# MisterPup/PDE-MultiGrid

Hardware: AMD Instinct MI355X
Metric: MLUPS on 3D Poisson 512^3 V-cycle (higher is better)
Workload: dtype f64

## Files before the change

include/mgx.h:

```cpp
#ifndef MGX_H
#define MGX_H

#include <stddef.h>
#include <stdint.h>

#ifdef __cplusplus
extern "C" {
#endif

typedef enum {
    MGX_OK = 0,
    MGX_ERR_INVALID = 1,
    MGX_ERR_SIZE = 2,
    MGX_ERR_HIP = 3,
    MGX_ERR_NOMEM = 4,
    MGX_ERR_RCCL = 5,
    MGX_ERR_NOGPU = 6
} mgx_status;

typedef enum { MGX_RESIDUAL_REF_COMPAT = 0, MGX_RESIDUAL_CORRECT = 1 } mgx_residual_mode;

typedef struct mgx_ctx mgx_ctx;
typedef struct mgx_event mgx_event;

const char* mgx_status_string(int status);
const char* mgx_last_error(void);
void mgx_set_last_error(const char* msg);
const char* mgx_version(void);

int mgx_device_count(int* count);
int mgx_ctx_create(int device, mgx_ctx** out);
int mgx_ctx_destroy(mgx_ctx* ctx);
int mgx_ctx_sync(mgx_ctx* ctx);
int mgx_ctx_check(mgx_ctx* ctx);
int mgx_ctx_clear_abort(mgx_ctx* ctx, int reenable);
int mgx_ctx_generation(const mgx_ctx* ctx, unsigned long long* generation);
int mgx_ctx_prepare(mgx_ctx* ctx);
int mgx_ctx_device(const mgx_ctx* ctx, int* device);
int mgx_ctx_set_param(mgx_ctx* ctx, const char* name, int value);
const char* mgx_ctx_last_relax_kernel(const mgx_ctx* ctx);
const char* mgx_ctx_last_rr_kernel(const mgx_ctx* ctx);
const char* mgx_ctx_last_corr_kernel(const mgx_ctx* ctx);
const char* mgx_ctx_last_block3_kernel(const mgx_ctx* ctx);
int mgx3dxs_relax_block3_f64(mgx_ctx* ctx, const double* vin, double* vout, const double* f, const int n[3], const double h[3],
                             int first_colour, int store_both);
int mgx3dxs_relax_block3_corr_f64(mgx_ctx* ctx, double* v, const double* f, const int n[3], const double h[3], const double* coarse_v,
                                  const int cn[3]);
int mgx_test_set_lds_poison(int on);
int mgx_test_lds_probe(mgx_ctx* ctx, double* fraction);
int mgx_ctx_stream(const mgx_ctx* ctx, void** hip_stream);

int mgx_malloc(mgx_ctx* ctx, size_t bytes, void** dptr);
int mgx_free(mgx_ctx* ctx, void* dptr);
int mgx_memcpy_h2d(mgx_ctx* ctx, void* dst, const void* host_src, size_t bytes);
int mgx_memcpy_d2h(mgx_ctx* ctx, void* host_dst, const void* src, size_t bytes);
int mgx_memcpy_d2d(mgx_ctx* ctx, void* dst, const void* src, size_t bytes);
int mgx_memset_zero(mgx_ctx* ctx, void* dst, size_t bytes);

int mgx_graph_begin(mgx_ctx* ctx);
int mgx_graph_end(mgx_ctx* ctx, void** graph_exec);
int mgx_graph_launch(mgx_ctx* ctx, void* graph_exec);
int mgx_graph_destroy(mgx_ctx* ctx, void* graph_exec);
int mgx_event_create(mgx_ctx* ctx, mgx_event** out);
int mgx_event_destroy(mgx_ctx* ctx, mgx_event* ev);
int mgx_event_record(mgx_ctx* ctx, mgx_event* ev);
int mgx_event_elapsed_ms(mgx_ctx* ctx, mgx_event* start, mgx_event* stop, float* ms);

#define MGX_DECLARE_OPS(SFX, real)                                                                      \
    int mgx3d_relax_##SFX(mgx_ctx* ctx, real* v, const real* f, const int n[3], const real h[3],        \
                          int ncycles);                                                                 \
     \
     \
     \
    int mgx3d_relax_from_zero_##SFX(mgx_ctx* ctx, real* v, const real* f, const int n[3], const real h[3], \
                                    int ncycles, int rim_is_zero);                                      \
    int mgx3d_residual_##SFX(mgx_ctx* ctx, const real* v, const real* f, real* r, const int n[3],       \
                             const real h[3], int mode);                                                \
    int mgx3d_restrict_##SFX(mgx_ctx* ctx, const real* fine, const int fn[3], real* coarse,             \
                             const int cn[3]);                                                          \
    int mgx3d_interpolate_##SFX(mgx_ctx* ctx, real* fine, const int fn[3], const real* coarse,          \
// ... 497 lines not shown
```

pde_multigrid_amd/csrc/mgx_block3d.hip:

```cpp
#include <type_traits>

#include "mgx_host3d.hpp"

namespace mgx {

template <class real, int COL, bool STORE_BOTH, int TW, bool CORR = false>
__global__ void __launch_bounds__(64 * TW, 4)
    relax3d_xs_block3_kernel(const real* vin, real* vout, const real* __restrict__ f, int sx, int sy, int sz, real hx2, real hy2,
                             real hz2, int zrun, int gx, int gy, int xcd_mode, const real* coarse = nullptr, int cx = 0,
                             int cy = 0) {
    constexpr int ROWS = 2 * TW, OUTR = ROWS - 6;
    static_assert(OUTR % 2 == 0, "the colour parity of a wave's rows must not depend on the tile");
    static_assert(!CORR || (COL == 0 && !STORE_BOTH), "the correcting variant is R', B, R with red stored");
    __shared__ real sY[2][TW][2][64];
    __shared__ real sX[2][TW][2][64];
    __shared__ real sZ[2][TW][2][64];
    const Geo<XSplit, real> g(sx, sy);
    const int lane = threadIdx.x;
    const int w = __builtin_amdgcn_readfirstlane(threadIdx.y);
    int bx, by, bz;
    tile_of_block(xcd_mode, gx, gy, bx, by, bz);
    const int z0 = 1 + bz * zrun, z1 = min(z0 + zrun, sz - 1);
    if (z0 >= z1) return;
    const int PL = (int)g.PL;

    const int Hn = (sx + 1) >> 1;
    const int pn = bx * 60 + lane - 2, p = min(max(pn, 0), Hn - 1);
    const unsigned off0 = (unsigned)p * (unsigned)sizeof(real), off1 = (unsigned)(g.H + (p <= Hn - 2 ? p : 0)) * (unsigned)sizeof(real);
    const bool xin0 = pn >= 1 && 2 * pn <= sx - 2, xin1 = pn >= 0 && 2 * pn + 1 <= sx - 2;
    auto off = [&](int h) { return h ? off1 : off0; };
    auto xin = [&](int h) { return h ? xin1 : xin0; };
    const bool xface0 = pn <= 0 || pn >= Hn - 1;
    const bool wxface = bx * 60 - 2 <= 0 || bx * 60 + 61 >= Hn - 1;
    const bool outlane = lane >= 2 && lane <= 61;
    int roff[2];
    bool yin[2], outrow[2];
#pragma unroll
    for (int o = 0; o < 2; o++) {
        const int y = by * OUTR - 3 + 2 * w + o;
        roff[o] = min(max(y, 0), sy - 1) * g.P;
        yin[o] = y >= 1 && y <= sy - 2;
        outrow[o] = 2 * w + o >= 3 && 2 * w + o < ROWS - 3;
    }
    const int wU = w > 0 ? w - 1 : 0, wD = w < TW - 1 ? w + 1 : TW - 1;
    auto zc = [&](int z) { return min(max(z, 0), sz - 1); };
    auto plane = [&](const real* a, int z) { return plane_rsrc<real>(a + (ptrdiff_t)zc(z) * (ptrdiff_t)g.PL, PL, 1); };
    const Geo<XSplit, real> gc(CORR ? cx : 3, CORR ? cy : 3);
    const int cz = (sz + 1) >> 1;
    int croff[2];
#pragma unroll
    for (int i = 0; i < 2; i++) croff[i] = CORR ? min(max(by * (OUTR / 2) - 2 + w + i, 0), cy - 1) * gc.P : 0;
    const unsigned coff = (unsigned)XSplit::pos(p, gc.H) * (unsigned)sizeof(real);
    auto cplane = [&](int k) {
        return plane_rsrc<real>(coarse + (ptrdiff_t)min(max(k, 0), cz - 1) * (ptrdiff_t)gc.PL, (int)gc.PL, 1);
    };
    auto interp = [&](int ox, int oz, int o, const real (&k0)[2], const real (&k1)[2]) __attribute__((always_inline)) {
        return interpolate3d_point<real>(ox, 1 - o, oz, [&](int dx, int dy, int dz) __attribute__((always_inline)) {
            const real c = o + dy ? (dz ? k1[1] : k0[1]) : (dz ? k1[0] : k0[0]);
            return dx ? wave_from_next_lane<real>(c) : c;
        });
    };

    real a_m[2], a_c[2], a_p[2], a_n[2], fx_c[2], fx_1[2], fx_2[2], fx_n[2], xv_n[2], fy_c[2], fy_n[2];
    real b_c[2], b_m[2], b_mm[2], d_c[2], d_m[2], d_mm[2], x3[2];
    real c_0[2], c_1[2], c_n[2], e_n[2];
#pragma unroll
    for (int o = 0; o < 2; o++)
        a_m[o] = a_c[o] = a_p[o] = a_n[o] = fx_c[o] = fx_1[o] = fx_2[o] = fx_n[o] = xv_n[o] = fy_c[o] = fy_n[o] = b_c[o] =
            b_m[o] = b_mm[o] = d_c[o] = d_m[o] = d_mm[o] = x3[o] = c_0[o] = c_1[o] = c_n[o] = e_n[o] = 0;

    const int t0 = z0 - 2, tlast = z1 + 1;
    {
        const auto qm = plane(vin, t0 - 1), q0 = plane(vin, t0), qp = plane(vin, t0 + 1);
        const bool zf = t0 <= 0 || t0 >= sz - 1;
        const auto qf = plane(f, t0);
#pragma unroll
        for (int o = 0; o < 2; o++) {
            const int hx = (COL + 1 + o + t0) & 1;
            a_m[o] = buf_load<real>(qm, off(hx), roff[o]);
            a_c[o] = buf_load<real>(q0, off(hx ^ 1), roff[o]);
            a_p[o] = buf_load<real>(qp, off(hx), roff[o]);
            fx_c[o] = buf_load<real>(zf || !yin[o] ? q0 : qf, off(hx), roff[o]);
            if (wxface) xv_n[o] = buf_load<real>(q0, off(0), roff[o]);
        }
        __builtin_amdgcn_s_waitcnt(0x0F70);
#pragma unroll
        for (int o = 0; o < 2; o++)
            if (wxface && ((COL + 1 + o + t0) & 1) == 0 && xface0) fx_c[o] = xv_n[o];
        if constexpr (CORR) {
#pragma unroll
            for (int d = -1; d <= 1; d++) {
                const int z = t0 + d;
                const auto k0q = cplane(z >> 1), k1q = cplane((z >> 1) + 1);
                real k0[2], k1[2];
#pragma unroll
                for (int i = 0; i < 2; i++) {
                    k0[i] = buf_load<real>(k0q, coff, croff[i]);
                    k1[i] = buf_load<real>(k1q, coff, croff[i]);
                }
                const bool zin = z >= 1 && z <= sz - 2;
#pragma unroll
                for (int o = 0; o < 2; o++) {
                    const int hb = (COL + o + z) & 1;
                    const real e = interp(hb, z & 1, o, k0, k1);
                    real& a = d < 0 ? a_m[o] : d == 0 ? a_c[o] : a_p[o];
// ... 13 lines not shown
        const int b = (t0 - 1) & 1;
        sY[b][w][0][lane] = a_c[0];
        sY[b][w][1][lane] = a_c[1];
        asm volatile("s_waitcnt lgkmcnt(0)\n\ts_barrier" ::: "memory");
    }

    auto relax = [&](auto hc, int o, const real (&c)[2], real nb, real sb, real D, real U, real fv) __attribute__((always_inline)) {
        constexpr int h = decltype(hc)::value;
        real O, E;
        if (h == 0) {
            O = wave_from_prev_lane<real>(c[o]);
            E = c[o];
        } else {
            O = c[o];
            E = wave_from_next_lane<real>(c[o]);
        }
        const real N = o == 0 ? nb : c[0], S = o == 1 ? sb : c[1];
        return relax3d_point<real>(O, E, N, S, D, U, fv, hx2, hy2, hz2);
    };

    auto iteration = [&](auto parity, int t) __attribute__((always_inline)) {
        constexpr int PAR = decltype(parity)::value;
        constexpr int PB = PAR ^ 1;
        const auto ro3 = plane(vout, t - 3), ro2 = plane(vout, t - 2);
        const auto rY = plane(vin, t + 2), rXv = plane(vin, t + 1), rFx = plane(f, t + 1), rFy = plane(f, t);
        const bool zf = t + 1 <= 0 || t + 1 >= sz - 1;
        __builtin_amdgcn_s_setprio(3);
#pragma unroll
        for (int o = 0; o < 2; o++) {
            const int hx = (COL + 1 + o + PAR) & 1;
            const bool sto = outlane && yin[o] && outrow[o];
            if (t - 3 >= z0 && t - 3 < z1 && sto && xin(hx ^ 1)) buf_store_nt<real>(x3[o], ro3, off(hx ^ 1), roff[o]);
            if (STORE_BOTH && t - 2 >= z0 && t - 2 < z1 && sto && xin(hx ^ 1)) buf_store_nt<real>(d_m[o], ro2, off(hx ^ 1), roff[o]);
            a_n[o] = buf_load<real>(rY, off(hx ^ 1), roff[o]);
            fx_n[o] = buf_load<real>(zf || !yin[o] ? rXv : rFx, off(hx ^ 1), roff[o]);
            if ((hx ^ 1) == 0 && wxface) xv_n[o] = buf_load<real>(rXv, off(0), roff[o]);
            fy_n[o] = buf_load<real>(rFy, off(hx ^ 1), roff[o]);
        }
        if constexpr (CORR && PAR == 0) {
            const auto qnc = cplane((t >> 1) + 3);
            __builtin_amdgcn_sched_barrier(0);
#pragma unroll
            for (int i = 0; i < 2; i++) c_n[i] = buf_load<real>(qnc, coff, croff[i]);
            __builtin_amdgcn_sched_barrier(0);
        }
        __builtin_amdgcn_s_setprio(0);
        const bool zin1 = t >= 1 && t <= sz - 2, zin2 = t - 1 >= 1 && t - 1 <= sz - 2;
        {
            const real nb = sY[PB][wU][1][lane], sb = sY[PB][wD][0][lane];
#pragma unroll
            for (int o = 0; o < 2; o++) {
                const real v1 = (((COL + 1 + PAR) & 1) ^ o) == 0
                                    ? relax(std::integral_constant<int, 0>{}, o, a_c, nb, sb, a_m[o], a_p[o], fx_c[o])
                                    : relax(std::integral_constant<int, 1>{}, o, a_c, nb, sb, a_m[o], a_p[o], fx_c[o]);
                const int hx = (COL + 1 + o + PAR) & 1;
                b_c[o] = zin1 && yin[o] && xin(hx) ? v1 : fx_c[o];
            }
        }
        {
            const real nb = sX[PB][wU][1][lane], sb = sX[PB][wD][0][lane];
#pragma unroll
            for (int o = 0; o < 2; o++) {
                const real v2 = (((COL + 1 + PAR) & 1) ^ o) == 0
                                    ? relax(std::integral_constant<int, 0>{}, o, b_m, nb, sb, b_mm[o], b_c[o], fy_c[o])
                                    : relax(std::integral_constant<int, 1>{}, o, b_m, nb, sb, b_mm[o], b_c[o], fy_c[o]);
                const int hx = (COL + 1 + o + PAR) & 1;
                d_c[o] = zin2 && yin[o] && xin(hx) ? v2 : a_m[o];
            }
        }
        {
            const real nb = sZ[PB][wU][1][lane], sb = sZ[PB][wD][0][lane];
#pragma unroll
            for (int o = 0; o < 2; o++) {
                x3[o] = (((COL + 1 + PAR) & 1) ^ o) == 0
                            ? relax(std::integral_constant<int, 0>{}, o, d_m, nb, sb, d_mm[o], d_c[o], fx_2[o])
                            : relax(std::integral_constant<int, 1>{}, o, d_m, nb, sb, d_mm[o], d_c[o], fx_2[o]);
            }
        }
        if constexpr (CORR) {
#pragma unroll
            for (int o = 0; o < 2; o++) e_n[o] = interp((COL + o + PAR) & 1, PAR, o, c_0, c_1);
        }
#pragma unroll
        for (int o = 0; o < 2; o++) {
            sY[PAR][w][o][lane] = a_p[o];
            sX[PAR][w][o][lane] = b_c[o];
            sZ[PAR][w][o][lane] = d_c[o];
        }
        asm volatile("s_waitcnt lgkmcnt(0)\n\ts_barrier" ::: "memory");
        if constexpr (CORR && PAR == 0) __builtin_amdgcn_s_waitcnt(0x0F72);
        else __builtin_amdgcn_s_waitcnt(0x0F70);
        const bool zin3 = t + 2 >= 1 && t + 2 <= sz - 2;
#pragma unroll
        for (int o = 0; o < 2; o++) {
            a_m[o] = a_c[o]; a_c[o] = a_p[o];
            a_p[o] = CORR && zin3 && yin[o] && xin((COL + o + PAR) & 1) ? a_n[o] + e_n[o] : a_n[o];
            if constexpr (CORR && PAR == 1) { c_0[o] = c_1[o]; c_1[o] = c_n[o]; }
            fx_2[o] = fx_1[o]; fx_1[o] = fx_c[o];
            fx_c[o] = ((COL + 1 + o + PAR) & 1) == 1 && wxface && xface0 ? xv_n[o] : fx_n[o];
            fy_c[o] = fy_n[o];
            b_mm[o] = b_m[o]; b_m[o] = b_c[o];
            d_mm[o] = d_m[o]; d_m[o] = d_c[o];
        }
    };

    int t = t0;
    if (t & 1) iteration(std::integral_constant<int, 1>{}, t++);
    for (;; t += 2) {
        iteration(std::integral_constant<int, 0>{}, t);
        if (t == tlast) break;
        iteration(std::integral_constant<int, 1>{}, t + 1);
        if (t + 1 == tlast) break;
    }
    {
        const auto ro3 = plane(vout, tlast - 2);
#pragma unroll
        for (int o = 0; o < 2; o++) {
            const int hx = (COL + 1 + o + tlast) & 1;
            if (outlane && yin[o] && outrow[o] && xin(hx)) buf_store_nt<real>(x3[o], ro3, off(hx), roff[o]);
        }
    }
}

bool relax_block3_takes(const mgx_ctx* ctx, const int n[3], size_t elem, int part) {
    if (!(ctx->block3 & part) || elem != 8) return false;
    if ((unsigned long long)Geo<XSplit, double>(n[0], n[1]).PL * 8ull >= (1ull << 31)) return false;
    return n[0] >= 385 && n[1] >= 129 && n[2] >= 65;
}

template <class real>
void relax3d_xs_block3_launch(mgx_ctx* ctx, const real* vin, real* vout, const real* f, const int n[3], real hx2, real hy2, real hz2,
                              int first_colour, bool store_both, const real* coarse, const int* cn) {
    constexpr int TW = 16;
    const int gx = ceil_div((n[0] - 1) / 2, 60), gy = ceil_div(n[1] - 2, 2 * TW - 6);
    const int tiles = gx * gy, planes = n[2] - 2;
    const int zrun = ceil_div(planes, runs_filling_rounds(tiles, planes, ctx->num_cus, 64, 16, 4));
    const dim3 grid(tiles * ceil_div(planes, zrun), 1, 1), blk(64, TW, 1);
#define MGX_B3(C, S)                                                                                                          \
    MGX_LAUNCH((relax3d_xs_block3_kernel<real, C, S, TW>), grid, blk, 0, ctx->compute, vin, vout, f, n[0], n[1], n[2], hx2, hy2, \
               hz2, zrun, gx, gy, 1)
    if (coarse) {
        MGX_LAUNCH((relax3d_xs_block3_kernel<real, 0, false, TW, true>), grid, blk, 0, ctx->compute, vin, vout, f, n[0], n[1], n[2], hx2,
                   hy2, hz2, zrun, gx, gy, 1, coarse, cn[0], cn[1]);
    } else if (first_colour == 0) {
        if (store_both) MGX_B3(0, true); else MGX_B3(0, false);
    } else {
        if (store_both) MGX_B3(1, true); else MGX_B3(1, false);
    }
#undef MGX_B3
    snprintf(ctx->last_block3_kernel, sizeof ctx->last_block3_kernel, "relax3d_xs_block3_kernel<%s,%d,%s,%d%s>",
             sizeof(real) == 8 ? "double" : "float", first_colour, store_both ? "true" : "false", TW, coarse ? ",corr" : "");
}
template void relax3d_xs_block3_launch<double>(mgx_ctx*, const double*, double*, const double*, const int[3], double, double, double, int,
                                               bool, const double*, const int*);
template <>
void relax3d_xs_block3_launch<float>(mgx_ctx*, const float*, float*, const float*, const int[3], float, float, float, int, bool, const float*,
                                     const int*) {}

}

extern "C" int mgx3dxs_relax_block3_f64(mgx_ctx* ctx, const double* vin, double* vout, const double* f, const int n[3], const double h[3],
                                        int first_colour, int store_both) {
    MGX_REQUIRE(ctx && vin && vout && f && n && h, MGX_ERR_INVALID, "relax_block3: NULL argument");
    MGX_USE(ctx);
    MGX_REQUIRE(mgx::valid_size(n[0]) && mgx::valid_size(n[1]) && mgx::valid_size(n[2]), MGX_ERR_SIZE,
                "relax_block3: sizes %d x %d x %d are not odd and >= 3", n[0], n[1], n[2]);
    MGX_REQUIRE(first_colour == 0 || first_colour == 1, MGX_ERR_INVALID, "relax_block3: first_colour = %d not in {0, 1}", first_colour);
    const unsigned long long plane_bytes = (unsigned long long)mgx::Geo<mgx::XSplit, double>(n[0], n[1]).PL * 8ull;
    MGX_REQUIRE(plane_bytes < (1ull << 31), MGX_ERR_SIZE,
                "relax_block3: a plane of %d x %d is too large", n[0], n[1]);
    MGX_REQUIRE(!store_both || vin != vout, MGX_ERR_INVALID, "relax_block3: store_both needs vout != vin");
    mgx::relax3d_xs_block3_launch<double>(ctx, vin, vout, f, n, h[0] * h[0], h[1] * h[1], h[2] * h[2], first_colour, store_both != 0, nullptr, nullptr);
    MGX_LAUNCH_CHECK();
    return MGX_OK;
}

extern "C" int mgx3dxs_relax_block3_corr_f64(mgx_ctx* ctx, double* v, const double* f, const int n[3], const double h[3], const double* coarse_v,
                                             const int cn[3]) {
    MGX_REQUIRE(ctx && v && f && n && h && coarse_v && cn, MGX_ERR_INVALID, "relax_block3_corr: NULL argument");
    MGX_USE(ctx);
    MGX_REQUIRE(mgx::valid_size(n[0]) && mgx::valid_size(n[1]) && mgx::valid_size(n[2]), MGX_ERR_SIZE,
                "relax_block3_corr: sizes %d x %d x %d are not odd and >= 3", n[0], n[1], n[2]);
    for (int d = 0; d < 3; d++)
        MGX_REQUIRE(cn[d] == (n[d] - 1) / 2 + 1, MGX_ERR_SIZE, "relax_block3_corr: coarse size[%d] = %d != (%d-1)/2+1", d, cn[d], n[d]);
    const unsigned long long plane_bytes = (unsigned long long)mgx::Geo<mgx::XSplit, double>(n[0], n[1]).PL * 8ull;
    MGX_REQUIRE(plane_bytes < (1ull << 31), MGX_ERR_SIZE, "relax_block3_corr: a plane of %d x %d is too large", n[0], n[1]);
    mgx::relax3d_xs_block3_launch<double>(ctx, v, v, f, n, h[0] * h[0], h[1] * h[1], h[2] * h[2], 0, false, coarse_v, cn);
    MGX_LAUNCH_CHECK();
    return MGX_OK;
}
```

pde_multigrid_amd/csrc/mgx_core.hip:

```cpp
#include "mgx_host3d.hpp"

namespace mgx {

static thread_local char g_err[1024] = "";

void set_error(const char* fmt, ...) {
    va_list ap;
    va_start(ap, fmt);
    vsnprintf(g_err, sizeof g_err, fmt, ap);
    va_end(ap);
}

typedef unsigned int u32x4 __attribute__((ext_vector_type(4)));
__global__ void __launch_bounds__(256) fill_zero_kernel(u32x4* __restrict__ p, size_t n16) {
    const u32x4 z = {0u, 0u, 0u, 0u};
    for (size_t i = (size_t)blockIdx.x * 256 + threadIdx.x; i < n16; i += (size_t)gridDim.x * 256) __builtin_nontemporal_store(z, &p[i]);
}

int fill_zero(mgx_ctx* ctx, void* dst, size_t bytes) {
    if (!bytes) return MGX_OK;
    if (bytes < ((size_t)4 << 20) || ((uintptr_t)dst & 15) || (bytes & 15)) {
        MGX_HIP(hipMemsetAsync(dst, 0, bytes, ctx->compute));
        return MGX_OK;
    }
// ... 420 lines not shown
        ctx->rr_black_waves = value;
    } else if (!strcmp(name, "rr3d.black_abl")) {
#ifdef MGX_DIAGNOSTICS
        ctx->rr_black_abl = value;
#else
        return mgx::fail(MGX_ERR_INVALID, "set_param: 'rr3d.black_abl' exists only in diagnostic builds (make diag)");
#endif
    } else if (!strcmp(name, "relax3d.fused_ilv")) {
        ctx->sweep_ilv = value ? 1 : 0;
    } else if (!strcmp(name, "relax3d.fused_mid")) {
        MGX_REQUIRE(value >= 0 && value <= 2, MGX_ERR_INVALID, "set_param: relax3d.fused_mid = %d not in {0, 1, 2}", value);
        ctx->sweep_mid = value;
    } else if (!strcmp(name, "relax3d.fused_dbg")) {
#ifdef MGX_DIAGNOSTICS
        ctx->sweep_dbg = value;
#else
        return mgx::fail(MGX_ERR_INVALID, "set_param: 'relax3d.fused_dbg' exists only in diagnostic builds (make diag)");
#endif
    } else if (!strcmp(name, "relax3d.fused_lead")) {
        MGX_REQUIRE(value == 0 || (value >= 5 && value <= 7), MGX_ERR_INVALID, "relax3d.fused_lead (planes the red stage runs ahead) must be 0 (default), 5, 6 or 7");
        ctx->sweep_lead = value;
    } else if (!strcmp(name, "relax3d.unroll")) {
        MGX_REQUIRE(value >= 0 && value <= 31, MGX_ERR_INVALID, "set_param: relax3d.unroll = %d not in [0, 31]", value);
        ctx->pipe_unroll = value;
    } else if (!strcmp(name, "relax3d.block3")) {
        MGX_REQUIRE(value == 0 || value == 1, MGX_ERR_INVALID, "set_param: relax3d.block3 = %d not in {0, 1}", value);
        ctx->block3 = (ctx->block3 & ~1) | value;
    } else if (!strcmp(name, "relax3d.block3_up")) {
        MGX_REQUIRE(value == 0 || value == 1, MGX_ERR_INVALID, "set_param: relax3d.block3_up = %d not in {0, 1}", value);
        ctx->block3 = (ctx->block3 & ~2) | (value << 1);
    } else if (!strcmp(name, "relax3d.block3_corr")) {
        MGX_REQUIRE(value == 0 || value == 1, MGX_ERR_INVALID, "set_param: relax3d.block3_corr = %d not in {0, 1}", value);
        ctx->block3 = (ctx->block3 & ~4) | (value << 2);
    } else if (!strcmp(name, "relax3d.zchunk")) {
        MGX_REQUIRE(value >= 0, MGX_ERR_INVALID, "relax3d.zchunk must be >= 0 (0 = automatic)");
        ctx->relax_zchunk = value;
    } else {
        return mgx::fail(MGX_ERR_INVALID, "set_param: unknown parameter '%s'", name);
    }
    return MGX_OK;
}

}
```

pde_multigrid_amd/csrc/mgx_host3d.hpp:

```cpp
#pragma once
#include "mgx_kernels3d.hpp"

namespace mgx {

#pragma GCC visibility push(hidden)

inline dim3 blk() { return dim3(64, 4, 1); }
inline dim3 grd(int nx, int ny, int nz) { return dim3(ceil_div(nx, 64), ceil_div(ny, 4), nz); }

inline int check_n3(const int n[3], const char* what) {
    MGX_REQUIRE(n, MGX_ERR_INVALID, "%s: size array is NULL", what);
    for (int d = 0; d < 3; d++)
        MGX_REQUIRE(valid_size(n[d]), MGX_ERR_SIZE, "%s: size[%d] = %d is not odd and >= 3", what, d, n[d]);
    MGX_REQUIRE((double)n[0] * n[1] * n[2] < 2147483647.0 * 4, MGX_ERR_SIZE, "%s: grid too large", what);
    return MGX_OK;
}

inline int check_coarse3(const int fn[3], const int cn[3], const char* what) {
    MGX_REQUIRE(fn && cn, MGX_ERR_INVALID, "%s: size array is NULL", what);
    for (int d = 0; d < 3; d++)
        MGX_REQUIRE(cn[d] == (fn[d] - 1) / 2 + 1, MGX_ERR_SIZE, "%s: coarse size[%d] = %d != (%d-1)/2+1", what, d, cn[d],
                    fn[d]);
    return MGX_OK;
}

inline int check_rr_args(mgx_ctx* ctx, bool nonnull, const int n[3], const int cn[3], const char* what) {
    MGX_REQUIRE(nonnull, MGX_ERR_INVALID, "%s: NULL argument", what);
    MGX_USE(ctx);
    MGX_TRY_RET(check_n3(n, what));
    return check_coarse3(n, cn, what);
}


bool relax3d_lds_shape_known(int shape);
template <class real>
int relax3d_xs_colour_passes(mgx_ctx* ctx, real* v, const real* f, const int n[3], const real h[3], int ncycles);
template <class real>
int relax3d_xs_from_zero(mgx_ctx* ctx, real* v, const real* f, const int n[3], const real h[3], int ncycles, int rim_is_zero);

enum class RRKernel { Window, Shuffle, Pipe, Black };
struct RRPlan {
    RRKernel kernel = RRKernel::Window;
    int T = 4, CR = 1, OWN = 4;
    int gx = 0, gy = 0, pzchunk = 0;
    dim3 grid, block;
    int xcd = 0;
};
bool rr_plan(const mgx_ctx* ctx, bool xsplit, bool black, const int n[3], const int cn[3], int planes, RRPlan& p);
template <class real, class L>
int residual_restrict3d(mgx_ctx* ctx, const real* v, const real* f, const int n[3], const real h[3], int mode, real* coarse_f,
                        const int cn[3], bool rim_is_zero = false);

bool relax_rr3d_xs_takes(const mgx_ctx* ctx, const int n[3], const int cn[3], size_t elem);
template <class real>
bool relax_rr3d_xs_launch(mgx_ctx* ctx, real* v, const real* f, const int n[3], const real h[3], int mode, real* coarse_f,
                          const int cn[3], int fzoff, int czoff, int pzbeg, int pzend);

bool relax_block3_takes(const mgx_ctx* ctx, const int n[3], size_t elem, int part);
template <class real>
void relax3d_xs_block3_launch(mgx_ctx* ctx, const real* vin, real* vout, const real* f, const int n[3], real hx2, real hy2, real hz2,
                              int first_colour, bool store_both, const real* coarse = nullptr, const int* cn = nullptr);
template <>
void relax3d_xs_block3_launch<float>(mgx_ctx*, const float*, float*, const float*, const int[3], float, float, float, int, bool, const float*,
                                     const int*);

struct SweepSync;
int sweep_state(mgx_ctx* ctx, SweepSync* out);
template <class real>
int relax3d_xs_pp(mgx_ctx* ctx, real* v, real* w, const real* f, const int n[3], const real h[3], int ncycles, int w_rim_valid);
template <class real>
void copy_rim3d_xs(mgx_ctx* ctx, const real* v, real* w, const int n[3]);

bool relax3d_resident_takes(const mgx_ctx* ctx, const int n[3], int ncycles);
template <class real>
int relax3d_resident(mgx_ctx* ctx, real* v, const real* f, const int n[3], real hx2, real hy2, real hz2, int ncycles, int zero_start);

int krylov_final(mgx_ctx* ctx, const double* work, size_t count, int nsums, double* dev_sum);
template <class real>
int cg_update3d(mgx_ctx* ctx, real* x, const real* p, real* r, const real* q, const int n[3], const double* dev_alpha, double* dev_work,
                double* dev_sum, bool finalize);
template <class real>
int dot2_3d(mgx_ctx* ctx, const real* a, const real* b, const real* c, const int n[3], double* dev_work, double* dev_sum, bool finalize);
template <class real>
int cg_direction3d(mgx_ctx* ctx, real* x, real* p, const real* z, const int n[3], const double* dev_alpha, const double* dev_beta);

#pragma GCC visibility pop

}
```

pde_multigrid_amd/csrc/mgx_internal.hpp:

```cpp
#pragma once
#include <hip/hip_runtime.h>

#include <cstdarg>
#include <cstdio>
#include <cstring>
#include <type_traits>

#include "mgx.h"

struct mgx_ctx {
    int device = 0;
    hipStream_t compute = nullptr;
    hipStream_t comm = nullptr;
    hipEvent_t ev_compute = nullptr;
    hipEvent_t ev_comm = nullptr;
    int comm_inline = 0;
    int relax_ty = 4;
    int relax_zchunk = 0;
    int relax_xcd = 1;
    int rr_rows = 0;
    int rr_rcp = 1;
    int mixed_fused = 0;
    int mixed_rows = 4;
    int mixed_zchunk = 0;
// ... 19 lines not shown
    int sweep_fused = 0;
    int sweep_mid = 1;
    int relax_resident = 1;
    int relax_resident_min = 3;
    void* resident_buf = nullptr;
    size_t resident_bytes = 0;
    int sweep_ilv = 0;
    int sweep_lead = 0;
    int sweep_dbg = 0;
    void* sweep_dev = nullptr;
    unsigned* sweep_abort = nullptr;
    unsigned sync_spin_limit = 1u << 21;
    unsigned handoff_fault = 0;
    int handoff_broken = 0;
    unsigned long long generation = 0;
    int gpu_exclusive = 1;
    mutable int resident_occ = -1;
    void* scratch = nullptr;
    size_t scratch_bytes = 0;
    void* rccl_comm = nullptr;
    void* local_group = nullptr;
    int rank = 0, nranks = 1;
    int comm_rehearse = 0;
    void* rehearse_buf = nullptr;
    size_t rehearse_bytes = 0;
    int num_cus = 256;
    int pipe_unroll = 7;
    int corr_low = 0;
    int slab_edges_merged = 1;
    int resident_tile = 0;
    char last_corr_kernel[96] = "";
    char last_rr_kernel[96] = "";
    char last_relax_kernel[96] = "";
    int block3 = 7;
    char last_block3_kernel[96] = "";
};

struct mgx_event {
    hipEvent_t ev = nullptr;
};

namespace mgx {

void set_error(const char* fmt, ...);

inline int fail(int status, const char* fmt, ...) {
    char buf[512];
    va_list ap;
    va_start(ap, fmt);
    vsnprintf(buf, sizeof buf, fmt, ap);
    va_end(ap);
    set_error("%s", buf);
    return status;
}

int workspace(mgx_ctx* ctx, size_t bytes, void** out);
int fill_zero(mgx_ctx* ctx, void* dst, size_t bytes);

inline int ceil_div(long long a, long long b) { return (int)((a + b - 1) / b); }

inline int runs_filling_rounds(long long tiles, int planes, long long slots, int max_runs, int min_run, int lead) {
    int runs = 1;
    double best = 0;
    for (int c = 1; c <= max_runs && (c == 1 || planes / c >= min_run); c++) {
        const long long wgs = tiles * c;
        double eff = (double)wgs / (double)(((wgs + slots - 1) / slots) * slots);
        if (lead > 0) eff = eff * (double)planes / (double)(planes + lead * c);
// ... 64 lines not shown
```

pde_multigrid_amd/csrc/mgx_kernels3d.hip:

```cpp
#include <type_traits>

#include "mgx_host3d.hpp"

namespace mgx {

template <class real>
__global__ void __launch_bounds__(256) relax3d_colour_kernel(real* __restrict__ v, const real* __restrict__ f, int sx,
                                                             int sy, int sz, real hx2, real hy2, real hz2, int colour) {
    const int y = 1 + blockIdx.y * blockDim.y + threadIdx.y;
    const int z = 1 + blockIdx.z;
    if (y >= sy - 1) return;
    const int p = (colour + y + z) & 1;
    const int x = 2 * (blockIdx.x * blockDim.x + threadIdx.x) + p;
    if (x < 1 || x >= sx - 1) return;
    const size_t sxy = (size_t)sx * sy;
    const size_t i = x + (size_t)y * sx + (size_t)z * sxy;
    const real O = v[i - 1], E = v[i + 1];
    const real N = v[i - sx], S = v[i + sx];
    const real D = v[i - sxy], U = v[i + sxy];
    v[i] = relax3d_point<real>(O, E, N, S, D, U, f[i], hx2, hy2, hz2);
}

template <class real, class L>
__global__ void __launch_bounds__(256) relax3d_zero_colour_kernel(real* __restrict__ v, const real* __restrict__ f, int sx, int sy,
// ... 2080 lines not shown
    const Geo<XSplit, real> ge(sx, sy);
    MGX_LAUNCH((set3d_kernel<real, XSplit>), grd(sx - 2, sy - 2, zend - zbeg), blk(), 0, ctx->compute,
                       g + ge.PL * (size_t)zbeg - ge.PL, sx, sy, zend - zbeg + 2, value, 1);
    MGX_LAUNCH_CHECK();
    return MGX_OK;
}

template <class real>
int relax_rr3d_slab(mgx_ctx* ctx, real* v, const real* f, const int n[3], int fzoff, const real h[3], int mode, real* coarse_f,
                    const int cn[3], int czoff, int pzbeg, int pzend) {
    MGX_TRY_RET(check_rr_args(ctx, ctx && v && f && h && coarse_f, n, cn, "relax_rr_slab"));
    MGX_REQUIRE(mode == MGX_RESIDUAL_REF_COMPAT || mode == MGX_RESIDUAL_CORRECT, MGX_ERR_INVALID, "relax_rr_slab: bad mode %d", mode);
    MGX_REQUIRE(pzbeg >= 1 && pzend <= cn[2] - 1 && pzbeg < pzend && czoff >= 0 && czoff <= pzbeg && fzoff >= 0 && (fzoff & 1) == 0 &&
                    fzoff <= (2 * pzbeg - 3 > 0 ? 2 * pzbeg - 3 : 0),
                MGX_ERR_INVALID, "relax_rr_slab: coarse planes [%d, %d) with offsets %d / %d", pzbeg, pzend, fzoff, czoff);
    MGX_REQUIRE(relax_rr3d_xs_takes(ctx, n, cn, sizeof(real)), MGX_ERR_INVALID, "relax_rr_slab: the level is not taken (ask relax_rr_takes)");
    const Geo<XSplit, real> gc(cn[0], cn[1]);
    MGX_TRY_RET(fill_zero(ctx, coarse_f + gc.PL * (size_t)(pzbeg - czoff), gc.PL * (size_t)(pzend - pzbeg) * sizeof(real)));
    MGX_REQUIRE(relax_rr3d_xs_launch<real>(ctx, v, f, n, h, mode, coarse_f, cn, fzoff, czoff, pzbeg, pzend), MGX_ERR_INVALID,
                "relax_rr_slab: launch refused");
    MGX_LAUNCH_CHECK();
    return MGX_OK;
}

template <class real>
int smooth_residual_restrict3d_xs(mgx_ctx* ctx, real* v, const real* f, const int n[3], const real h[3], int ncycles, int from_zero,
                                  int v_rim_is_zero, int mode, real* coarse_f, const int cn[3], int coarse_rim_is_zero) {
    MGX_TRY_RET(check_rr_args(ctx, ctx && v && f && h && coarse_f, n, cn, "smooth_residual_restrict3d"));
    MGX_REQUIRE(ncycles >= 0, MGX_ERR_INVALID, "smooth_residual_restrict3d: ncycles = %d < 0", ncycles);
    MGX_REQUIRE(mode == MGX_RESIDUAL_REF_COMPAT || mode == MGX_RESIDUAL_CORRECT, MGX_ERR_INVALID,
                "smooth_residual_restrict3d: bad mode %d", mode);
    ctx->last_rr_kernel[0] = 0;
    ctx->last_block3_kernel[0] = 0;
    if (ncycles < 1 || !relax_rr3d_xs_takes(ctx, n, cn, sizeof(real))) {
        MGX_TRY_RET((from_zero ? relax3d_from_zero<real, XSplit>(ctx, v, f, n, h, ncycles, v_rim_is_zero) : relax3d<real, XSplit>(ctx, v, f, n, h, ncycles)));
        return residual_restrict3d<real, XSplit>(ctx, v, f, n, h, mode, coarse_f, cn, coarse_rim_is_zero != 0);
    }
    const real hx2 = h[0] * h[0], hy2 = h[1] * h[1], hz2 = h[2] * h[2];
    int s = 0;
    if (from_zero) {
        if (v_rim_is_zero && ctx->relax_zero_first) {
            if (2 * ncycles - 1 >= 2 && relax3d_xs_first_sweep_zero<real>(ctx, v, f, n[0], n[1], n[2], hx2, hy2, hz2)) {
                s = 2;
            } else {
                MGX_LAUNCH((relax3d_zero_colour_kernel<real, XSplit>), dim3(ceil_div((n[0] + 1) / 2, 64), ceil_div(n[1] - 2, 4), n[2] - 2),
                                   blk(), 0, ctx->compute, v, f, n[0], n[1], hx2, hy2, hz2, 0, 1);
                s = 1;
            }
        } else {
            MGX_TRY_RET(fill_zero(ctx, v, Geo<XSplit, real>(n[0], n[1]).PL * (size_t)n[2] * sizeof(real)));
        }
    }
    const bool b3 = !from_zero && 2 * ncycles - 1 - s >= 3 && relax_block3_takes(ctx, n, sizeof(real), 1);
    for (; s < 2 * ncycles - 1 - (b3 ? 3 : 0); s++) relax3d_xs_pass<real>(ctx, v, f, n[0], n[1], 1, n[2] - 1, hx2, hy2, hz2, s & 1);
    if (b3) relax3d_xs_block3_launch<real>(ctx, v, v, f, n, hx2, hy2, hz2, 0, false);
    if (!coarse_rim_is_zero) MGX_TRY_RET(fill_zero(ctx, coarse_f, Geo<XSplit, real>(cn[0], cn[1]).PL * (size_t)cn[2] * sizeof(real)));
    MGX_REQUIRE(relax_rr3d_xs_launch<real>(ctx, v, f, n, h, mode, coarse_f, cn, 0, 0, 1, cn[2] - 1), MGX_ERR_INVALID,
                "smooth_residual_restrict3d: the fused launch refused a level it had accepted");
    MGX_LAUNCH_CHECK();
    return MGX_OK;
}

template <class real, class L>
int init_f3d(mgx_ctx* ctx, real* f, const int n[3], double c, const double* tx, const double* ty, const double* tz) {
    MGX_REQUIRE(ctx && f && tx && ty && tz, MGX_ERR_INVALID, "init_f3d: NULL argument");
    MGX_USE(ctx);
    int st = check_n3(n, "init_f3d");
    if (st) return st;
    const size_t cnt = (size_t)n[0] + n[1] + n[2];
    void* ws = nullptr;
    st = workspace(ctx, cnt * sizeof(double), &ws);
    if (st) return st;
    double* d = (double*)ws;
    MGX_HIP(hipMemcpyAsync(d, tx, n[0] * sizeof(double), hipMemcpyHostToDevice, ctx->compute));
    MGX_HIP(hipMemcpyAsync(d + n[0], ty, n[1] * sizeof(double), hipMemcpyHostToDevice, ctx->compute));
    MGX_HIP(hipMemcpyAsync(d + n[0] + n[1], tz, n[2] * sizeof(double), hipMemcpyHostToDevice, ctx->compute));
    MGX_LAUNCH((init_f3d_kernel<real, L>), grd(n[0], n[1], n[2]), blk(), 0, ctx->compute, f, n[0], n[1], n[2], c, d,
                       d + n[0], d + n[0] + n[1]);
    MGX_LAUNCH_CHECK();
    MGX_HIP(hipStreamSynchronize(ctx->compute));
    return MGX_OK;
}

template <class real, class LS, class LD>
int relayout3d(mgx_ctx* ctx, const real* src, real* dst, const int n[3]) {
    MGX_REQUIRE(ctx && src && dst, MGX_ERR_INVALID, "relayout3d: NULL argument");
    MGX_USE(ctx);
    MGX_REQUIRE(src != dst, MGX_ERR_INVALID, "relayout3d: in-place conversion is not supported");
// ... 547 lines not shown
```

pde_multigrid_amd/multigrid.py:

```python
import ctypes as C

import numpy as np

from ._lib import CORRECT, REF_COMPAT, check, lib


def _ct(dtype):
    dtype = np.dtype(dtype)
    if dtype == np.float32:
        return "f32", C.c_float
    if dtype == np.float64:
        return "f64", C.c_double
    raise TypeError("dtype must be float32 or float64, got %s" % dtype)


def _ip(a):
    return (C.c_int * len(a))(*[int(x) for x in a])


def _rp(a, ct):
    return (ct * len(a))(*[float(x) for x in a])


def _shape(n):
# ... 339 lines not shown

    def smooth_residual_restrict(self, ctx, v, f, n, rng, ncycles, from_zero=False, v_rim_is_zero=False, mode=REF_COMPAT, dtype=None):
        dtype = dtype or v.dtype
        fn, ct = self._fn("smooth_residual_restrict", dtype)
        h = _rp(grid_spacing(n, rng, dtype), ct)
        cn = coarse_size(n)
        pv, pf = ctx.to_device(xs_pack(np.ascontiguousarray(v, dtype))), ctx.to_device(xs_pack(np.ascontiguousarray(f, dtype)))
        pc = ctx.to_device(xs_pack(np.full(_shape(cn), np.nan, dtype)))
        try:
            check(fn(ctx._h, pv, pf, _ip(n), h, C.c_int(ncycles), C.c_int(int(from_zero)), C.c_int(int(v_rim_is_zero)), C.c_int(mode), pc,
                     _ip(cn), C.c_int(0)))
            isz = np.dtype(dtype).itemsize
            out_v = xs_unpack(ctx.to_host(pv, tuple(_shape(n)[:-1]) + (xs_geometry(n[0], isz)[1],), dtype), n[0])
            out_c = xs_unpack(ctx.to_host(pc, tuple(_shape(cn)[:-1]) + (xs_geometry(cn[0], isz)[1],), dtype), cn[0])
            return out_v, out_c
        finally:
            for q in (pv, pf, pc):
                ctx.free(q)

    def relax_block3(self, ctx, vin, f, n, rng, first_colour=0, store_both=False, vout=None):
        h = _rp(grid_spacing(n, rng, np.float64), C.c_double)
        arrs = [vin, f] if vout is None else [vin, f, vout]
        if vout is None:
            call = lambda a, b: lib.mgx3dxs_relax_block3_f64(ctx._h, a, a, b, _ip(n), h, C.c_int(first_colour), C.c_int(int(store_both)))
            return self._run(ctx, arrs, call, 0, _shape(n), np.float64)
        call = lambda a, b, c: lib.mgx3dxs_relax_block3_f64(ctx._h, a, c, b, _ip(n), h, C.c_int(first_colour), C.c_int(int(store_both)))
        return self._run(ctx, arrs, call, 2, _shape(n), np.float64)

    def relax_block3_corr(self, ctx, v, f, n, rng, coarse):
        h = _rp(grid_spacing(n, rng, np.float64), C.c_double)
        cn = coarse_size(n)
        return self._run(ctx, [v, f, coarse], lambda a, b, c: lib.mgx3dxs_relax_block3_corr_f64(ctx._h, a, b, _ip(n), h, c, _ip(cn)), 0,
                         _shape(n), np.float64)

    def interpolate_correct_relax_block3(self, ctx, v, f, n, rng, coarse, ncycles, dtype=None):
        dtype = dtype or v.dtype
        fn, ct = self._fn("interpolate_correct_relax_block3", dtype)
        h = _rp(grid_spacing(n, rng, dtype), ct)
        cn = coarse_size(n)
        return self._run(ctx, [v, f, coarse], lambda a, b, c: fn(ctx._h, a, b, _ip(n), h, c, _ip(cn), C.c_int(ncycles)), 0, _shape(n),
                         dtype)

    def interpolate_correct_relax(self, ctx, v, f, n, rng, coarse, ncycles, dtype=None):
        dtype = dtype or v.dtype
        fn, ct = self._fn("interpolate_correct_relax", dtype)
        h = _rp(grid_spacing(n, rng, dtype), ct)
        cn = coarse_size(n)
        return self._run(ctx, [v, f, coarse], lambda a, b, c: fn(ctx._h, a, b, _ip(n), h, c, _ip(cn), C.c_int(ncycles)), 0, _shape(n),
                         dtype)

    def jacobi(self, ctx, v, f, n, rng, omega, ncycles, dtype=None):
        dtype = dtype or v.dtype
        fn, ct = self._fn("jacobi", dtype)
        h = _rp(grid_spacing(n, rng, dtype), ct)
        return self._run(ctx, [v, np.zeros_like(v), f], lambda a, t, b: fn(ctx._h, a, t, b, _ip(n), h, ct(omega), C.c_int(ncycles)),
                         0, _shape(n), dtype)

    def norm2(self, ctx, x):
        s, _ = _ct(x.dtype)
        out = C.c_double()
        p = ctx.to_device(x)
        try:
            check(getattr(lib, "mgx_norm2_" + s)(ctx._h, p, C.c_size_t(x.size), C.byref(out)))
        finally:
            ctx.free(p)
        return float(out.value)
# ... 1065 lines not shown
```

Baseline: 240,800.

## Add from-zero block3 kernel fusing the first three sweeps when v starts at zero

Adds a ZERO variant of the three-colour block3 relax kernel. Because v is known to be zero, it skips every load of v, the first red update reduces to a pure f term, and the variant is used as the first three sweeps of smooth_residual_restrict on downward levels. It also lowers the size threshold for block3 variants from 385 to 257 so more levels qualify, and adds a fallback path when the fused residual-restrict is not taken. This removes separate passes and v reads on the pre-smoothing of each level, at the cost of another kernel instantiation and more branching in the host dispatch.

```diff
diff --git a/include/mgx.h b/include/mgx.h
--- a/include/mgx.h
+++ b/include/mgx.h
@@ -46,6 +46,8 @@
                              int first_colour, int store_both);
 int mgx3dxs_relax_block3_corr_f64(mgx_ctx* ctx, double* v, const double* f, const int n[3], const double h[3], const double* coarse_v,
                                   const int cn[3]);
+int mgx3dxs_relax_block3_zero_f64(mgx_ctx* ctx, double* v, const double* f, const int n[3], const double h[3]);
+int mgx3dxs_block3_zero_takes_f64(const mgx_ctx* ctx, const int n[3], int ncycles);
 int mgx_test_set_lds_poison(int on);
 int mgx_test_lds_probe(mgx_ctx* ctx, double* fraction);
 int mgx_ctx_stream(const mgx_ctx* ctx, void** hip_stream);
diff --git a/pde_multigrid_amd/csrc/mgx_block3d.hip b/pde_multigrid_amd/csrc/mgx_block3d.hip
--- a/pde_multigrid_amd/csrc/mgx_block3d.hip
+++ b/pde_multigrid_amd/csrc/mgx_block3d.hip
@@ -4,7 +4,7 @@
 
 namespace mgx {
 
-template <class real, int COL, bool STORE_BOTH, int TW, bool CORR = false>
+template <class real, int COL, bool STORE_BOTH, int TW, bool CORR = false, bool ZERO = false>
 __global__ void __launch_bounds__(64 * TW, 4)
     relax3d_xs_block3_kernel(const real* vin, real* vout, const real* __restrict__ f, int sx, int sy, int sz, real hx2, real hy2,
                              real hz2, int zrun, int gx, int gy, int xcd_mode, const real* coarse = nullptr, int cx = 0,
@@ -12,6 +12,7 @@
     constexpr int ROWS = 2 * TW, OUTR = ROWS - 6;
     static_assert(OUTR % 2 == 0, "the colour parity of a wave's rows must not depend on the tile");
     static_assert(!CORR || (COL == 0 && !STORE_BOTH), "the correcting variant is R', B, R with red stored");
+    static_assert(!ZERO || (COL == 0 && !STORE_BOTH && !CORR), "the from-zero variant is R0, B, R with red stored");
     __shared__ real sY[2][TW][2][64];
     __shared__ real sX[2][TW][2][64];
     __shared__ real sZ[2][TW][2][64];
@@ -70,7 +71,12 @@
             b_m[o] = b_mm[o] = d_c[o] = d_m[o] = d_mm[o] = x3[o] = c_0[o] = c_1[o] = c_n[o] = e_n[o] = 0;
 
     const int t0 = z0 - 2, tlast = z1 + 1;
-    {
+    if constexpr (ZERO) {
+        const auto qf = plane(f, t0);
+#pragma unroll
+        for (int o = 0; o < 2; o++) fx_c[o] = buf_load<real>(qf, off((COL + 1 + o + t0) & 1), roff[o]);
+        __builtin_amdgcn_s_waitcnt(0x0F70);
+    } else {
         const auto qm = plane(vin, t0 - 1), q0 = plane(vin, t0), qp = plane(vin, t0 + 1);
         const bool zf = t0 <= 0 || t0 >= sz - 1;
         const auto qf = plane(f, t0);
@@ -150,9 +156,9 @@
             const bool sto = outlane && yin[o] && outrow[o];
             if (t - 3 >= z0 && t - 3 < z1 && sto && xin(hx ^ 1)) buf_store_nt<real>(x3[o], ro3, off(hx ^ 1), roff[o]);
             if (STORE_BOTH && t - 2 >= z0 && t - 2 < z1 && sto && xin(hx ^ 1)) buf_store_nt<real>(d_m[o], ro2, off(hx ^ 1), roff[o]);
-            a_n[o] = buf_load<real>(rY, off(hx ^ 1), roff[o]);
-            fx_n[o] = buf_load<real>(zf || !yin[o] ? rXv : rFx, off(hx ^ 1), roff[o]);
-            if ((hx ^ 1) == 0 && wxface) xv_n[o] = buf_load<real>(rXv, off(0), roff[o]);
+            if constexpr (!ZERO) a_n[o] = buf_load<real>(rY, off(hx ^ 1), roff[o]);
+            fx_n[o] = buf_load<real>(!ZERO && (zf || !yin[o]) ? rXv : rFx, off(hx ^ 1), roff[o]);
+            if (!ZERO && (hx ^ 1) == 0 && wxface) xv_n[o] = buf_load<real>(rXv, off(0), roff[o]);
             fy_n[o] = buf_load<real>(rFy, off(hx ^ 1), roff[o]);
         }
         if constexpr (CORR && PAR == 0) {
@@ -164,7 +170,14 @@
         }
         __builtin_amdgcn_s_setprio(0);
         const bool zin1 = t >= 1 && t <= sz - 2, zin2 = t - 1 >= 1 && t - 1 <= sz - 2;
-        {
+        if constexpr (ZERO) {
+            const real zero = (real)0;
+#pragma unroll
+            for (int o = 0; o < 2; o++) {
+                const real v1 = relax3d_point<real>(zero, zero, zero, zero, zero, zero, fx_c[o], hx2, hy2, hz2);
+                b_c[o] = zin1 && yin[o] && xin((COL + 1 + o + PAR) & 1) ? v1 : zero;
+            }
+        } else {
             const real nb = sY[PB][wU][1][lane], sb = sY[PB][wD][0][lane];
 #pragma unroll
             for (int o = 0; o < 2; o++) {
@@ -201,7 +214,7 @@
         }
 #pragma unroll
         for (int o = 0; o < 2; o++) {
-            sY[PAR][w][o][lane] = a_p[o];
+            if constexpr (!ZERO) sY[PAR][w][o][lane] = a_p[o];
             sX[PAR][w][o][lane] = b_c[o];
             sZ[PAR][w][o][lane] = d_c[o];
         }
@@ -215,7 +228,7 @@
             a_p[o] = CORR && zin3 && yin[o] && xin((COL + o + PAR) & 1) ? a_n[o] + e_n[o] : a_n[o];
             if constexpr (CORR && PAR == 1) { c_0[o] = c_1[o]; c_1[o] = c_n[o]; }
             fx_2[o] = fx_1[o]; fx_1[o] = fx_c[o];
-            fx_c[o] = ((COL + 1 + o + PAR) & 1) == 1 && wxface && xface0 ? xv_n[o] : fx_n[o];
+            fx_c[o] = !ZERO && ((COL + 1 + o + PAR) & 1) == 1 && wxface && xface0 ? xv_n[o] : fx_n[o];
             fy_c[o] = fy_n[o];
             b_mm[o] = b_m[o]; b_m[o] = b_c[o];
             d_mm[o] = d_m[o]; d_m[o] = d_c[o];
@@ -240,15 +253,24 @@
     }
 }
 
+static int block3_min_row(const mgx_ctx* ctx, int part) {
+    const int i = part == 1 ? 0 : part == 2 ? 1 : part == 4 ? 2 : 3;
+    static const int rule[4] = {BLOCK3_MIN_DOWN, BLOCK3_MIN_UP, BLOCK3_MIN_CORR, BLOCK3_MIN_ZERO};
+    return ctx->block3_min[i] ? ctx->block3_min[i] : rule[i];
+}
 bool relax_block3_takes(const mgx_ctx* ctx, const int n[3], size_t elem, int part) {
     if (!(ctx->block3 & part) || elem != 8) return false;
     if ((unsigned long long)Geo<XSplit, double>(n[0], n[1]).PL * 8ull >= (1ull << 31)) return false;
-    return n[0] >= 385 && n[1] >= 129 && n[2] >= 65;
+    return n[0] >= block3_min_row(ctx, part) && n[1] >= 129 && n[2] >= 65;
+}
+
+bool block3_zero_takes(const mgx_ctx* ctx, const int n[3], size_t elem, int ncycles) {
+    return ncycles == 2 && ctx->relax_zero_first && relax_block3_takes(ctx, n, elem, 8);
 }
 
 template <class real>
 void relax3d_xs_block3_launch(mgx_ctx* ctx, const real* vin, real* vout, const real* f, const int n[3], real hx2, real hy2, real hz2,
-                              int first_colour, bool store_both, const real* coarse, const int* cn) {
+                              int first_colour, bool store_both, const real* coarse, const int* cn, bool zero) {
     constexpr int TW = 16;
     const int gx = ceil_div((n[0] - 1) / 2, 60), gy = ceil_div(n[1] - 2, 2 * TW - 6);
     const int tiles = gx * gy, planes = n[2] - 2;
@@ -260,6 +282,9 @@
     if (coarse) {
         MGX_LAUNCH((relax3d_xs_block3_kernel<real, 0, false, TW, true>), grid, blk, 0, ctx->compute, vin, vout, f, n[0], n[1], n[2], hx2,
                    hy2, hz2, zrun, gx, gy, 1, coarse, cn[0], cn[1]);
+    } else if (zero) {
+        MGX_LAUNCH((relax3d_xs_block3_kernel<real, 0, false, TW, false, true>), grid, blk, 0, ctx->compute, vin, vout, f, n[0], n[1], n[2],
+                   hx2, hy2, hz2, zrun, gx, gy, 1);
     } else if (first_colour == 0) {
         if (store_both) MGX_B3(0, true); else MGX_B3(0, false);
     } else {
@@ -267,13 +292,13 @@
     }
 #undef MGX_B3
     snprintf(ctx->last_block3_kernel, sizeof ctx->last_block3_kernel, "relax3d_xs_block3_kernel<%s,%d,%s,%d%s>",
-             sizeof(real) == 8 ? "double" : "float", first_colour, store_both ? "true" : "false", TW, coarse ? ",corr" : "");
+             sizeof(real) == 8 ? "double" : "float", first_colour, store_both ? "true" : "false", TW, coarse ? ",corr" : zero ? ",zero" : "");
 }
 template void relax3d_xs_block3_launch<double>(mgx_ctx*, const double*, double*, const double*, const int[3], double, double, double, int,
-                                               bool, const double*, const int*);
+                                               bool, const double*, const int*, bool);
 template <>
 void relax3d_xs_block3_launch<float>(mgx_ctx*, const float*, float*, const float*, const int[3], float, float, float, int, bool, const float*,
-                                     const int*) {}
+                                     const int*, bool) {}
 
 }
 
@@ -307,3 +332,19 @@
     MGX_LAUNCH_CHECK();
     return MGX_OK;
 }
+
+extern "C" int mgx3dxs_relax_block3_zero_f64(mgx_ctx* ctx, double* v, const double* f, const int n[3], const double h[3]) {
+    MGX_REQUIRE(ctx && v && f && n && h, MGX_ERR_INVALID, "relax_block3_zero: NULL argument");
+    MGX_USE(ctx);
+    MGX_REQUIRE(mgx::valid_size(n[0]) && mgx::valid_size(n[1]) && mgx::valid_size(n[2]), MGX_ERR_SIZE,
+                "relax_block3_zero: sizes %d x %d x %d are not odd and >= 3", n[0], n[1], n[2]);
+    const unsigned long long plane_bytes = (unsigned long long)mgx::Geo<mgx::XSplit, double>(n[0], n[1]).PL * 8ull;
+    MGX_REQUIRE(plane_bytes < (1ull << 31), MGX_ERR_SIZE, "relax_block3_zero: a plane of %d x %d is too large", n[0], n[1]);
+    mgx::relax3d_xs_block3_launch<double>(ctx, v, v, f, n, h[0] * h[0], h[1] * h[1], h[2] * h[2], 0, false, nullptr, nullptr, true);
+    MGX_LAUNCH_CHECK();
+    return MGX_OK;
+}
+
+extern "C" int mgx3dxs_block3_zero_takes_f64(const mgx_ctx* ctx, const int n[3], int ncycles) {
+    return ctx && n && mgx::block3_zero_takes(ctx, n, 8, ncycles);
+}
diff --git a/pde_multigrid_amd/csrc/mgx_core.hip b/pde_multigrid_amd/csrc/mgx_core.hip
--- a/pde_multigrid_amd/csrc/mgx_core.hip
+++ b/pde_multigrid_amd/csrc/mgx_core.hip
@@ -476,6 +476,13 @@
     } else if (!strcmp(name, "relax3d.block3_corr")) {
         MGX_REQUIRE(value == 0 || value == 1, MGX_ERR_INVALID, "set_param: relax3d.block3_corr = %d not in {0, 1}", value);
         ctx->block3 = (ctx->block3 & ~4) | (value << 2);
+    } else if (!strcmp(name, "relax3d.block3_zero")) {
+        MGX_REQUIRE(value == 0 || value == 1, MGX_ERR_INVALID, "set_param: relax3d.block3_zero = %d not in {0, 1}", value);
+        ctx->block3 = (ctx->block3 & ~8) | (value << 3);
+    } else if (!strcmp(name, "relax3d.block3_min") || !strcmp(name, "relax3d.block3_up_min") || !strcmp(name, "relax3d.block3_corr_min") ||
+               !strcmp(name, "relax3d.block3_zero_min")) {
+        MGX_REQUIRE(value >= 0, MGX_ERR_INVALID, "set_param: %s = %d < 0", name, value);
+        ctx->block3_min[!strcmp(name, "relax3d.block3_min") ? 0 : !strcmp(name, "relax3d.block3_up_min") ? 1 : !strcmp(name, "relax3d.block3_corr_min") ? 2 : 3] = value;
     } else if (!strcmp(name, "relax3d.zchunk")) {
         MGX_REQUIRE(value >= 0, MGX_ERR_INVALID, "relax3d.zchunk must be >= 0 (0 = automatic)");
         ctx->relax_zchunk = value;
diff --git a/pde_multigrid_amd/csrc/mgx_host3d.hpp b/pde_multigrid_amd/csrc/mgx_host3d.hpp
--- a/pde_multigrid_amd/csrc/mgx_host3d.hpp
+++ b/pde_multigrid_amd/csrc/mgx_host3d.hpp
@@ -56,13 +56,15 @@
 bool relax_rr3d_xs_launch(mgx_ctx* ctx, real* v, const real* f, const int n[3], const real h[3], int mode, real* coarse_f,
                           const int cn[3], int fzoff, int czoff, int pzbeg, int pzend);
 
+constexpr int BLOCK3_MIN_DOWN = 257, BLOCK3_MIN_UP = 257, BLOCK3_MIN_CORR = 257, BLOCK3_MIN_ZERO = 257;
 bool relax_block3_takes(const mgx_ctx* ctx, const int n[3], size_t elem, int part);
+bool block3_zero_takes(const mgx_ctx* ctx, const int n[3], size_t elem, int ncycles);
 template <class real>
 void relax3d_xs_block3_launch(mgx_ctx* ctx, const real* vin, real* vout, const real* f, const int n[3], real hx2, real hy2, real hz2,
-                              int first_colour, bool store_both, const real* coarse = nullptr, const int* cn = nullptr);
+                              int first_colour, bool store_both, const real* coarse = nullptr, const int* cn = nullptr, bool zero = false);
 template <>
 void relax3d_xs_block3_launch<float>(mgx_ctx*, const float*, float*, const float*, const int[3], float, float, float, int, bool, const float*,
-                                     const int*);
+                                     const int*, bool);
 
 struct SweepSync;
 int sweep_state(mgx_ctx* ctx, SweepSync* out);
diff --git a/pde_multigrid_amd/csrc/mgx_internal.hpp b/pde_multigrid_amd/csrc/mgx_internal.hpp
--- a/pde_multigrid_amd/csrc/mgx_internal.hpp
+++ b/pde_multigrid_amd/csrc/mgx_internal.hpp
@@ -75,7 +75,8 @@
     char last_corr_kernel[96] = "";
     char last_rr_kernel[96] = "";
     char last_relax_kernel[96] = "";
-    int block3 = 7;
+    int block3 = 15;
+    int block3_min[4] = {0, 0, 0, 0};
     char last_block3_kernel[96] = "";
 };
 
diff --git a/pde_multigrid_amd/csrc/mgx_kernels3d.hip b/pde_multigrid_amd/csrc/mgx_kernels3d.hip
--- a/pde_multigrid_amd/csrc/mgx_kernels3d.hip
+++ b/pde_multigrid_amd/csrc/mgx_kernels3d.hip
@@ -2136,15 +2136,22 @@
                 "smooth_residual_restrict3d: bad mode %d", mode);
     ctx->last_rr_kernel[0] = 0;
     ctx->last_block3_kernel[0] = 0;
-    if (ncycles < 1 || !relax_rr3d_xs_takes(ctx, n, cn, sizeof(real))) {
+    const bool rr = ncycles >= 1 && relax_rr3d_xs_takes(ctx, n, cn, sizeof(real));
+    const bool bz = from_zero && v_rim_is_zero && block3_zero_takes(ctx, n, sizeof(real), ncycles);
+    const bool b1 = !bz && 2 * ncycles - 1 >= 3 && relax_block3_takes(ctx, n, sizeof(real), 1);
+    if (!rr && !bz && !b1) {
         MGX_TRY_RET((from_zero ? relax3d_from_zero<real, XSplit>(ctx, v, f, n, h, ncycles, v_rim_is_zero) : relax3d<real, XSplit>(ctx, v, f, n, h, ncycles)));
         return residual_restrict3d<real, XSplit>(ctx, v, f, n, h, mode, coarse_f, cn, coarse_rim_is_zero != 0);
     }
     const real hx2 = h[0] * h[0], hy2 = h[1] * h[1], hz2 = h[2] * h[2];
+    const int last = 2 * ncycles - 1;
     int s = 0;
-    if (from_zero) {
+    if (bz) {
+        relax3d_xs_block3_launch<real>(ctx, v, v, f, n, hx2, hy2, hz2, 0, false, nullptr, nullptr, true);
+        s = 3;
+    } else if (from_zero) {
         if (v_rim_is_zero && ctx->relax_zero_first) {
-            if (2 * ncycles - 1 >= 2 && relax3d_xs_first_sweep_zero<real>(ctx, v, f, n[0], n[1], n[2], hx2, hy2, hz2)) {
+            if (last >= 2 && relax3d_xs_first_sweep_zero<real>(ctx, v, f, n[0], n[1], n[2], hx2, hy2, hz2)) {
                 s = 2;
             } else {
                 MGX_LAUNCH((relax3d_zero_colour_kernel<real, XSplit>), dim3(ceil_div((n[0] + 1) / 2, 64), ceil_div(n[1] - 2, 4), n[2] - 2),
@@ -2155,9 +2162,14 @@
             MGX_TRY_RET(fill_zero(ctx, v, Geo<XSplit, real>(n[0], n[1]).PL * (size_t)n[2] * sizeof(real)));
         }
     }
-    const bool b3 = !from_zero && 2 * ncycles - 1 - s >= 3 && relax_block3_takes(ctx, n, sizeof(real), 1);
-    for (; s < 2 * ncycles - 1 - (b3 ? 3 : 0); s++) relax3d_xs_pass<real>(ctx, v, f, n[0], n[1], 1, n[2] - 1, hx2, hy2, hz2, s & 1);
+    const bool b3 = b1 && last - s >= 3;
+    for (; s < last - (b3 ? 3 : 0); s++) relax3d_xs_pass<real>(ctx, v, f, n[0], n[1], 1, n[2] - 1, hx2, hy2, hz2, s & 1);
     if (b3) relax3d_xs_block3_launch<real>(ctx, v, v, f, n, hx2, hy2, hz2, 0, false);
+    if (!rr) {
+        relax3d_xs_pass<real>(ctx, v, f, n[0], n[1], 1, n[2] - 1, hx2, hy2, hz2, 1);
+        MGX_LAUNCH_CHECK();
+        return residual_restrict3d<real, XSplit>(ctx, v, f, n, h, mode, coarse_f, cn, coarse_rim_is_zero != 0);
+    }
     if (!coarse_rim_is_zero) MGX_TRY_RET(fill_zero(ctx, coarse_f, Geo<XSplit, real>(cn[0], cn[1]).PL * (size_t)cn[2] * sizeof(real)));
     MGX_REQUIRE(relax_rr3d_xs_launch<real>(ctx, v, f, n, h, mode, coarse_f, cn, 0, 0, 1, cn[2] - 1), MGX_ERR_INVALID,
                 "smooth_residual_restrict3d: the fused launch refused a level it had accepted");
diff --git a/pde_multigrid_amd/multigrid.py b/pde_multigrid_amd/multigrid.py
--- a/pde_multigrid_amd/multigrid.py
+++ b/pde_multigrid_amd/multigrid.py
@@ -395,6 +395,13 @@
         cn = coarse_size(n)
         return self._run(ctx, [v, f, coarse], lambda a, b, c: lib.mgx3dxs_relax_block3_corr_f64(ctx._h, a, b, _ip(n), h, c, _ip(cn)), 0,
                          _shape(n), np.float64)
+
+    def relax_block3_zero(self, ctx, v, f, n, rng):
+        h = _rp(grid_spacing(n, rng, np.float64), C.c_double)
+        return self._run(ctx, [v, f], lambda a, b: lib.mgx3dxs_relax_block3_zero_f64(ctx._h, a, b, _ip(n), h), 0, _shape(n), np.float64)
+
+    def block3_zero_takes(self, ctx, n, ncycles):
+        return bool(lib.mgx3dxs_block3_zero_takes_f64(ctx._h, _ip(n), C.c_int(ncycles)))
 
     def interpolate_correct_relax_block3(self, ctx, v, f, n, rng, coarse, ncycles, dtype=None):
         dtype = dtype or v.dtype
```

Result: no change. 243,600 (median of 6 runs) (+1.2%).
